# facebookresearch/theseus

Measured on NVIDIA H100. Metric: LM iterations/sec on batched SE3 pose-graph (2500 poses, global batch 2048 over N GPUs, LM + block-sparse Cholesky, fp64), higher is better.
Workload: dtype f64

## Files before the change

### include/thb200.h

```cpp
#ifndef THB200_H_
#define THB200_H_

#include <stdint.h>

#ifdef __cplusplus
extern "C" {
#endif

typedef struct CUstream_st* thb_stream_t;

#define THB_OK 0
#define THB_ERR_BAD_ARG (-1)
#define THB_ERR_UNSUPPORTED (-2)
#define THB_ERR_ALLOC (-3)

int thb_version(void);
int thb_compiled_arch(void);
int64_t thb_launch_count(void);

enum thb_cost_kind {
  THB_COST_BETWEEN_SE3 = 0,
  THB_COST_LOCAL_SE3 = 1,
  THB_COST_BETWEEN_SO3 = 2,
  THB_COST_LOCAL_SO3 = 3,
// ... 260 lines not shown
                       const float* err_prev, const float* err_new, float* lam, int32_t ellipsoidal, float damping_accept,
                       float down_ratio, float up_ratio, uint8_t* reject, float* err_out, int32_t* stats, thb_stream_t stream);

int thb_gram_dense_f64(const double* A, double* AtA, int64_t B, int64_t m, int64_t n, thb_stream_t stream);

typedef struct thb_front_plan {
  int64_t S;
  int64_t n;
  int64_t data_size;
  int64_t arena_size;
  int64_t varena_size;
  const int32_t* f_w; const int32_t* f_b; const int32_t* f_first; const int32_t* f_class;
  const int32_t* f_wpad; const int32_t* f_np; const int32_t* f_cb_ld; const int32_t* f_depth;
  const int64_t* f_panel_off; const int64_t* f_cb_off; const int64_t* f_fr_off; const int64_t* f_u_off;
  const int32_t* child_ptr; const int32_t* child_list;
  const int64_t* rel_ptr; const int32_t* f_rel;
  const int64_t* rows_ptr; const int32_t* f_rows;
  const int32_t* sched;
  const int32_t* perm;
  const int32_t* c_jw; const int64_t* c_sp_ptr; const int32_t* c_sp;
  const int64_t* c_inv_ptr; const int32_t* c_inv;
  const int64_t* fd; const int64_t* pc;
  const int32_t* pmap;
} thb_front_plan;

#define THB_FRONT_LAUNCH_COLS 12
int64_t thb_front_small_smem_bytes(int32_t w, int32_t b, int32_t nchildren);
int thb_front_factor_f64(const thb_front_plan* p, const int64_t* launches, int64_t num_launches, double* factor, const double* ata,
                         int64_t ata_stride, const double* alpha, const double* beta, double* arena, void* dense_ws, int64_t dense_ws_bytes,
                         int32_t* info, int64_t B, thb_stream_t stream);
int thb_front_solve_f64(const thb_front_plan* p, const int64_t* launches, int64_t num_launches, const double* factor, const double* rhs,
                        double* x, double* work, double* varena, int64_t B, thb_stream_t stream);
int thb_front_factor_forward_f64(const thb_front_plan* p, const int64_t* launches, int64_t num_launches, double* factor, const double* ata,
                                 int64_t ata_stride, const double* alpha, const double* beta, double* arena, void* dense_ws,
                                 int64_t dense_ws_bytes, int32_t* info, const double* rhs, double* work, double* varena, int64_t B,
                                 thb_stream_t stream);
int thb_front_forward_f64(const thb_front_plan* p, const int64_t* launches, int64_t num_launches, const double* factor, const double* rhs,
                          double* work, double* varena, int64_t B, thb_stream_t stream);
int thb_front_backward_f64(const thb_front_plan* p, const int64_t* launches, int64_t num_launches, const double* factor, double* x,
                           double* work, int64_t B, thb_stream_t stream);
int64_t thb_potrf_partial_workspace_bytes(int64_t B, int64_t np);
int thb_potrf_partial_inplace_f64(double* F, int64_t bstride, int64_t np, int32_t nb_piv, int32_t w_real, int32_t n_real, int32_t info_base,
                                  int32_t* info, int64_t B, void* workspace, int64_t workspace_bytes, thb_stream_t stream);

int thb_mat_vec_f64(int64_t B, int64_t num_rows, int64_t num_cols, const int64_t* row_ptr, const int64_t* col_ind,
                    const double* A_val, const double* v, double* y, thb_stream_t stream);
// ... 49 lines not shown
```

### theseus_b200/_lib.py

```python
import ctypes as C
import os

_HERE = os.path.dirname(os.path.abspath(__file__))
_LIB_PATH = os.environ.get("THB200_LIB") or os.path.join(_HERE, "lib", "libthb200.so")
_lib = None

c_i32, c_i64, c_f64, c_f32, c_vp = C.c_int32, C.c_int64, C.c_double, C.c_float, C.c_void_p


class CostGroup(C.Structure):
    _fields_ = [("kind", c_i32), ("weight_kind", c_i32), ("K", c_i32), ("dim", c_i32),
                ("x0", c_vp), ("x1", c_vp), ("aux", c_vp), ("w", c_vp), ("bstride", c_vp),
                ("a_off", c_vp), ("a_stride", c_vp), ("bp", c_vp), ("row0", c_vp),
                ("aux2", c_vp), ("aux3", c_vp), ("aux4", c_vp), ("bstride2", c_vp),
                ("robust_kind", c_i32), ("reserved0", c_i32), ("log_radius", c_vp), ("bstride_lr", c_vp),
                ("x2", c_vp), ("x3", c_vp), ("bstride3", c_vp), ("grid_rows", c_i32), ("grid_cols", c_i32)]


class VarTable(C.Structure):
    _fields_ = [("N", c_i32), ("x", c_vp), ("out", c_vp), ("kind", c_vp), ("col", c_vp), ("dof", c_vp)]


_GRAM_STAGED = ("stage_ptr", "st_off", "st_len", "st_row0", "st_dim", "st_soff", "task_ptr", "task_blk", "task_pq", "grp_col", "c_soff",
                "cc_soff", "cc_sb")
# ... 41 lines not shown

_PG, _PV, _PP = C.POINTER(CostGroup), C.POINTER(VarTable), C.POINTER(GramPlan)
_PS = C.POINTER(SparsePlanStruct)
_PL = C.POINTER(SparseLanePlanStruct)


class SparseLaneRootStruct(C.Structure):
    _fields_ = [("num_blocks", c_i64), ("num_cols", c_i64), ("nt", c_i64), ("root_start", c_i64), ("num_segments", c_i64)] + [(k, c_vp) for k in (
        "segments", "rb_off", "rb_row", "rb_col", "rb_di", "rb_dj", "rf_p0", "rf_p1", "root_cols", "root_dims")]


class SparseLaneTilesStruct(C.Structure):
    _fields_ = [("num_tiles", c_i64), ("num_steps", c_i64), ("tile_tgt", c_vp), ("step_ptr", c_vp), ("step_src", c_vp)]


class SparseLanePiecesStruct(C.Structure):
    _fields_ = [("num_pieces", c_i64), ("num_launches", c_i64)] + [(k, c_vp) for k in (
        "launches", "first", "width", "fr_ext_end", "bc_int_end", "order")]


class FrontPlanStruct(C.Structure):
    _fields_ = [("S", c_i64), ("n", c_i64), ("data_size", c_i64), ("arena_size", c_i64), ("varena_size", c_i64)] + [(k, c_vp) for k in (
        "f_w", "f_b", "f_first", "f_class", "f_wpad", "f_np", "f_cb_ld", "f_depth", "f_panel_off", "f_cb_off", "f_fr_off", "f_u_off",
        "child_ptr", "child_list", "rel_ptr", "f_rel", "rows_ptr", "f_rows", "sched", "perm", "c_jw", "c_sp_ptr", "c_sp", "c_inv_ptr", "c_inv", "fd", "pc", "pmap")]


_PF = C.POINTER(FrontPlanStruct)
_PR = C.POINTER(SparseLaneRootStruct)
_PPIECES = C.POINTER(SparseLanePiecesStruct)
_PT = C.POINTER(SparseLaneTilesStruct)
SIGNATURES = {
    "thb_version": (c_i32, []),
    "thb_compiled_arch": (c_i32, []),
    "thb_launch_count": (c_i64, []),
    "thb_linearize_group_f64": (c_i32, [_PG, c_i64, c_vp, c_i64, c_vp, c_i64, c_vp]),
    "thb_linearize_group_f32": (c_i32, [_PG, c_i64, c_vp, c_i64, c_vp, c_i64, c_vp]),
    "thb_error_num_chunks": (c_i32, [c_i32]),
    "thb_error_group_f64": (c_i32, [_PG, c_i64, c_vp, c_vp]),
    "thb_error_group_f32": (c_i32, [_PG, c_i64, c_vp, c_vp]),
    "thb_error_reduce_f64": (c_i32, [c_vp, c_i32, c_i64, c_vp, c_vp]),
    "thb_error_reduce_f32": (c_i32, [c_vp, c_i32, c_i64, c_vp, c_vp]),
    "thb_retract_f64": (c_i32, [_PV, c_i64, c_vp, c_i64, c_f64, c_vp, c_vp]),
    "thb_retract_f32": (c_i32, [_PV, c_i64, c_vp, c_i64, c_f32, c_vp, c_vp]),
    "thb_commit_f64": (c_i32, [_PV, c_i64, c_vp, c_vp]),
    "thb_commit_f32": (c_i32, [_PV, c_i64, c_vp, c_vp]),
    "thb_gram_f64": (c_i32, [_PP, c_i64, c_vp, c_i64, c_vp, c_i64, c_vp, c_i64, c_vp, c_vp, c_vp]),
    "thb_gram_f32": (c_i32, [_PP, c_i64, c_vp, c_i64, c_vp, c_i64, c_vp, c_i64, c_vp, c_vp, c_vp]),
# ... 104 lines not shown
```

### theseus_b200/csrc/thb_front.cu

```cuda
#include <stdlib.h>

#include "thb_common.cuh"

namespace thb {

__device__ __forceinline__ void record_first_failure(int* info, int pos) {
  int old = 0;
  while (true) {
    const int prev = atomicCAS(info, old, pos);
    if (prev == old || (prev != 0 && prev <= pos)) return;
    old = prev;
  }
}

#ifdef THB_SIMT_EMU
#define THB_PDL_TRIGGER() do { } while (0)
#define THB_PDL_WAIT() do { } while (0)
#define FRONT_LAUNCH(K, grid, block, smem, cs, arg) K<<<grid, block, smem, cs>>>(arg)
#else
#define THB_PDL_TRIGGER() asm volatile("griddepcontrol.launch_dependents;" ::: "memory")
#define THB_PDL_WAIT() asm volatile("griddepcontrol.wait;" ::: "memory")
#define FRONT_LAUNCH(K, grid, block, smem, cs, arg) thb::front_launch_pdl(K, grid, block, smem, cs, arg)
static inline bool front_pdl_enabled() {
  static const bool on = [] { const char* e = getenv("THB_FRONT_PDL"); return e != nullptr && e[0] == '1'; }();
// ... 27 lines not shown
  asm volatile("mma.sync.aligned.m8n8k4.row.col.f64.f64.f64.f64 {%0,%1}, {%2}, {%3}, {%0,%1};\n" : "+d"(c0), "+d"(c1) : "d"(a), "d"(b));
}
#endif

__host__ __device__ __forceinline__ int front_pad_ld(int x) { return ((x + 11) / 16) * 16 + 4; }

struct FrontArgs {
  thb_front_plan p;
  int s0;
  int64_t B;
  double* factor;
  const double* alpha;
  const double* beta;
  double* arena_cur;
  const double* arena_child;
  int32_t* info;
  int prefetch;
  const double* ata;
  int64_t ata_stride;
  const double* rhs;
  double* work;
  double* v_cur;
  const double* v_child;
};

__device__ __forceinline__ double front_panel_in(const FrontArgs& a, const double* Lg, int64_t poff, int64_t item, int64_t e) {
  if (a.ata == nullptr) return Lg[e];
  const int32_t m = a.p.pmap[poff + e];
  return m >= 0 ? a.ata[item * a.ata_stride + m] : 0.0;
}

template <typename T>
__device__ __forceinline__ T front_ldg(const T* p) {
#ifdef THB_SIMT_EMU
  return *p;
#else
  return __ldg(p);
#endif
}


constexpr int FRONT_WD_LD = 20;
#ifndef FRONT_PL
#define FRONT_PL 4
#endif
constexpr int FRONT_MAX_CHILDREN = 8;

// ... 230 lines not shown
    i += di; j += dj;
    if (j >= w) { j -= w; i++; }
  }
}

__device__ __forceinline__ void front_store_forward(const FrontArgs& a, const double* U, int ldp, int64_t item, int t, int f_first, int w, int b,
                                                    int tid, int nthreads) {
  for (int i = tid; i < w; i += nthreads) a.work[item * a.p.n + f_first + i] = U[i * ldp];
  double* ub = a.v_cur + item * a.p.varena_size + a.p.f_u_off[t];
  for (int i = tid; i < b; i += nthreads) ub[i] = U[(w + i) * ldp];
}

__host__ __device__ constexpr int front_elim_warps(int threads) { return threads >= 256 ? 4 : threads / 64; }

template <int THREADS>
__global__ void __launch_bounds__(THREADS, 1024 / THREADS) front_small_kernel(FrontArgs a) {
  extern __shared__ double sm[];
  const thb_front_plan& p = a.p;
  const int tid = threadIdx.x, lane = tid & 31, warp = tid >> 5;
  constexpr int NW = THREADS / 32;
  const int lr = lane >> 2, lc = lane & 3;
  const int64_t item = blockIdx.x;
  THB_PDL_TRIGGER();
  const int64_t* FD = p.fd + (int64_t)(a.s0 + blockIdx.y) * 8;
  const int t = (int)FD[0];
  const int w = (int)FD[1], b = (int)FD[2], r = w + b;
  const int f_first = (int)FD[3];
  const int64_t f_panel_off = FD[4];
  const int c_begin = (int)(FD[7] & 0xffffffffLL);
  const int nch = min((int)(FD[7] >> 32), FRONT_MAX_CHILDREN);
  const int b16 = (b + 15) & ~15, w8 = (w + 7) & ~7;
  const int ldp = front_pad_ld(w8);
  const int prow = w8 + b16 + 8;
  double* PN = sm;
  double* Wd = PN + prow * ldp;
  FrontChild* ch = reinterpret_cast<FrontChild*>(Wd + 8 * FRONT_WD_LD);
  int32_t* INV = reinterpret_cast<int32_t*>(Wd + 8 * FRONT_WD_LD + 3 * FRONT_MAX_CHILDREN);
  if (tid < nch) {
    const int64_t* PC = p.pc + (int64_t)(c_begin + tid) * 6;
    ch[tid].src = a.arena_child + item * p.arena_size + PC[0];
    ch[tid].ldg = (int)(PC[1] & 0xffffffffLL);
    ch[tid].lo = (int)PC[2];
    ch[tid].hi = (int)PC[3];
    ch[tid].uoff = (int)PC[5];
  }
  {
// ... 13 lines not shown
  int* next_tile = reinterpret_cast<int*>(Wd + 8);
  if (tid == 0) *next_tile = 0;
  THB_PDL_WAIT();
#ifndef THB_SIMT_EMU
  if (a.rhs != nullptr) {
    for (int i = tid; i < w; i += THREADS) asm volatile("prefetch.global.L2 [%0];\n" ::"l"(a.rhs + item * p.n + p.perm[f_first + i]));
    for (int q = 0; q < nch; q++) {
      const int64_t* PC = p.pc + (int64_t)(c_begin + q) * 6;
      const double* cu = a.v_child + item * p.varena_size + PC[5];
      for (int off = tid * 16; off < (int)(PC[1] >> 32); off += THREADS * 16) asm volatile("prefetch.global.L2 [%0];\n" ::"l"(cu + off));
    }
  }
  for (int q = 0; a.prefetch != 0 && q < nch; q++) {
    const int64_t* PC = p.pc + (int64_t)(c_begin + q) * 6;
    const double* csrc = a.arena_child + item * p.arena_size + PC[0];
    const int cld = (int)(PC[1] & 0xffffffffLL), cbc = (int)(PC[1] >> 32);
    for (int off = tid * 16; off < cbc * cld; off += THREADS * 16) {
      const int i = off / cld, j = off - i * cld;
      if (j <= i) asm volatile("prefetch.global.L2 [%0];\n" ::"l"(csrc + off));
    }
  }
#endif
  __syncthreads();
  if (tid < w8 - w) PN[(w + tid) * ldp + w + tid] = 1.0;
  double* Lg = a.factor + item * p.data_size + f_panel_off;
  {
    const double al = a.alpha != nullptr ? a.alpha[item] : 0.0;
    const double be = a.beta != nullptr ? a.beta[item] : 0.0;
    const int total = r * w;
    for (int e0 = tid; e0 < total; e0 += FRONT_PL * THREADS) {
      int ii[FRONT_PL], jj[FRONT_PL];
      double v[FRONT_PL];
#pragma unroll
      for (int u = 0; u < FRONT_PL; u++) {
        const int e = e0 + u * THREADS;
        ii[u] = e / w;
        jj[u] = e - ii[u] * w;
        if (e >= total || jj[u] > ii[u]) ii[u] = -1;
      }
      int32_t m[FRONT_PL];
#pragma unroll
      for (int u = 0; u < FRONT_PL; u++) m[u] = (a.ata != nullptr && ii[u] >= 0) ? front_ldg(p.pmap + f_panel_off + e0 + u * THREADS) : -1;
      double x[2][FRONT_PL];
      front_panel_gather2(ch, INV, r, nch, 0, ii, jj, x);
#pragma unroll
      for (int u = 0; u < FRONT_PL; u++) {
        if (a.ata != nullptr) v[u] = m[u] >= 0 ? front_ldg(a.ata + item * a.ata_stride + m[u]) : 0.0;
        else v[u] = ii[u] >= 0 ? Lg[e0 + u * THREADS] : 0.0;
      }
#pragma unroll
      for (int u = 0; u < FRONT_PL; u++)
        if (ii[u] >= 0 && ii[u] == jj[u]) v[u] = v[u] + (al * v[u] + be);
      for (int q = 0;;) {
#pragma unroll
        for (int u = 0; u < FRONT_PL; u++) v[u] = (v[u] + x[0][u]) + x[1][u];
        q += 2;
        if (q >= nch) break;
        front_panel_gather2(ch, INV, r, nch, q, ii, jj, x);
      }
#pragma unroll
      for (int u = 0; u < FRONT_PL; u++)
        if (ii[u] >= 0) PN[(ii[u] < w ? ii[u] : ii[u] + (w8 - w)) * ldp + jj[u]] = v[u];
    }
  }
  double* U = PN + w8;
  if (a.rhs != nullptr) {
    for (int i = tid; i < r; i += THREADS) {
      double v = i < w ? a.rhs[item * p.n + p.perm[f_first + i]] : 0.0;
      for (int q = 0; q < nch; q++) {
        if (i >= ch[q].lo && i <= ch[q].hi) {
          const int k = INV[q * r + i];
          if (k >= 0) v += a.v_child[item * p.varena_size + ch[q].uoff + k];
        }
      }
      U[i * ldp] = v;
    }
  }
  __syncthreads();
  const int nbk = w8 / 8, nrt = (w8 + b16) / 8;
  for (int jb = 0; jb < nbk; jb++) {
    if (warp == 0) front_diag_block(PN, ldp, jb, Wd, lane, w, f_first, a.info + item);
    __syncthreads();
    const int npair = (nrt - jb) / 2;
    for (int q = warp; q < npair; q += NW) front_tile_column<true>(PN, ldp, jb, jb + 1 + 2 * q, Wd, lane);
    __syncthreads();
  }
#ifdef THB_SIMT_EMU
  front_store_panel(Lg, PN, ldp, w, w8, r, tid, THREADS);
  if (a.rhs != nullptr) {
    front_forward_elim<THREADS, true>(FrontRowsPanel{PN, ldp, w, w8 - w}, U, ldp, w, r, tid, lane);
    front_store_forward(a, U, ldp, item, t, f_first, w, b, tid, THREADS);
  }
#else
  constexpr int NE = front_elim_warps(THREADS);
  if (a.rhs != nullptr && warp < NE) {
    front_forward_elim<32 * NE, false>(FrontRowsPanel{PN, ldp, w, w8 - w}, U, ldp, w, r, tid, lane);
    front_store_forward(a, U, ldp, item, t, f_first, w, b, tid, 32 * NE);
  } else {
    const int t0 = a.rhs != nullptr ? 32 * NE : 0;
    front_store_panel(Lg, PN, ldp, w, w8, r, tid - t0, THREADS - t0);
  }
#endif
  if (b == 0) return;
  double* dst = a.arena_cur + item * p.arena_size + FD[5];
  const int ldg_out = (int)FD[6];
  const double* P = PN + w8 * ldp;
  const int nmt = b16 / 16;
  for (;;) {
    int q = 0;
    if (lane == 0) q = atomicAdd(next_tile, 1);
    q = __shfl_sync(0xffffffffu, q, 0);
    int R = (int)((sqrtf(8.0f * (float)q + 1.0f) - 1.0f) * 0.5f);
    while ((R + 1) * (R + 2) / 2 <= q) R++;
    while (R * (R + 1) / 2 > q) R--;
    if (R >= nmt) break;
    const int ct = q - R * (R + 1) / 2;
    unsigned reach = 0;
    for (int qc = 0; qc < nch; qc++)
      if (w + 16 * R + 15 >= ch[qc].lo && w + 16 * ct <= ch[qc].hi) reach |= 1u << qc;
    double gch[2][2][2] = {{{-0.0, -0.0}, {-0.0, -0.0}}, {{-0.0, -0.0}, {-0.0, -0.0}}};
    const int li0 = w + 16 * R + lr, lj0 = w + 16 * ct + 2 * lc;
    if (reach != 0) {
      const int qc = front_next_child(reach);
      front_tile_gather(ch[qc], INV + qc * r, r, li0, lj0, gch);
    }
    const bool summed = reach != 0;
// ... 32 lines not shown
          for (int u = 0; u < 2; u++) gch[mi][ni][u] = 0.0 + gch[mi][ni][u];
    }
#pragma unroll
    for (int mi = 0; mi < 2; mi++)
#pragma unroll
      for (int ni = 0; ni < 2; ni++)
#pragma unroll
        for (int u = 0; u < 2; u++) acc[mi][ni][u] = gch[mi][ni][u] - acc[mi][ni][u];
#pragma unroll
    for (int mi = 0; mi < 2; mi++) {
      const int i = 16 * R + 8 * mi + lr;
      if (i < b) {
        double* drow = dst + (int64_t)i * ldg_out;
#pragma unroll
        for (int ni = 0; ni < 2; ni++)
#pragma unroll
          for (int u = 0; u < 2; u++) {
            const int jj = 16 * ct + 8 * ni + 2 * lc + u;
            if (jj <= i) drow[jj] = acc[mi][ni][u];
          }
      }
    }
  }
}

constexpr int ASM_ROWS = 16, ASM_THREADS = 256;

__device__ __forceinline__ int front_map_big(int l, int w, int wpad) { return l < w ? l : wpad + (l - w); }

__global__ void __launch_bounds__(ASM_THREADS, 4) front_assemble_kernel(FrontArgs a, int t) {
  extern __shared__ double sm[];
  const thb_front_plan& p = a.p;
  const int tid = threadIdx.x;
  const int64_t item = blockIdx.x;
  const int w = p.f_w[t], b = p.f_b[t], r = w + b, wpad = p.f_wpad[t], np = p.f_np[t];
  const int R0 = blockIdx.y * ASM_ROWS;
  const int nc = min(np, 128 * (R0 / 128 + 1));
  const int c_first = p.child_ptr[t], n_children = p.child_ptr[t + 1] - c_first;
  if (n_children <= FRONT_MAX_CHILDREN) {
    const double* Lgg = a.factor + item * p.data_size + p.f_panel_off[t];
    const double alg = a.alpha != nullptr ? a.alpha[item] : 0.0;
    const double beg = a.beta != nullptr ? a.beta[item] : 0.0;
    double* Fg = a.arena_cur + item * p.arena_size + p.f_fr_off[t] + (int64_t)R0 * np;
    __shared__ const double* s_src[FRONT_MAX_CHILDREN];
    __shared__ const int32_t* s_inv[FRONT_MAX_CHILDREN];
    __shared__ int s_ld[FRONT_MAX_CHILDREN];
// ... 261 lines not shown
    __syncthreads();
    if (warp == 0) {
      double tk = 0.0;
      if (lane < cw) {
        tk = xf[k0 + lane];
        for (int g = 0; g < RG; g++) tk -= part[g * cw + lane];
      }
      tk = front_warp_trsv_upper(T, tk, cw, lane);
      if (lane < cw) xf[k0 + lane] = tk;
    }
    __syncthreads();
  }
  for (int i = tid; i < w; i += THREADS) {
    const double v = xf[i];
    wk[first + i] = v;
    a.x[item * p.n + p.perm[first + i]] = v;
  }
}

static inline bool front_big_direct() {
  const char* e = getenv("THB_FRONT_BIG_DIRECT");
  return !(e != nullptr && e[0] == '0');
}

static inline int front_threads_of_class(int cls) { return cls == 0 ? 64 : (cls == 1 ? 128 : 256); }

template <typename K>
static inline int front_set_smem(K kernel, size_t bytes, size_t* cache) {
  if (bytes > *cache) {
    cudaError_t e = cudaFuncSetAttribute(kernel, cudaFuncAttributeMaxDynamicSharedMemorySize, (int)bytes);
    if (e != cudaSuccess) return (int)e;
    *cache = bytes;
  }
  return 0;
}

static int front_solve_launch(const thb_front_plan* p, const int64_t* L, int pass, const double* factor, const double* rhs, double* x,
                              double* work, double* varena, int64_t B, cudaStream_t cs) {
  static size_t fw_set[3] = {0, 0, 0}, bw_set[3] = {0, 0, 0};
  static const int64_t stage_cap = [] { const char* e = getenv("THB_SOLVE_STAGE"); return e != nullptr ? (int64_t)atoll(e) : (int64_t)0; }();
  const int depth = (int)L[0], cls = (int)L[1], begin = (int)L[2], count = (int)L[3];
  FrontSolveArgs a;
  a.p = *p; a.s0 = begin; a.B = B; a.factor = factor; a.rhs = rhs; a.x = x; a.work = work;
  a.v_cur = varena != nullptr ? varena + (int64_t)(depth & 1) * B * p->varena_size : nullptr;
  a.v_child = varena != nullptr ? varena + (int64_t)((depth + 1) & 1) * B * p->varena_size : nullptr;
  const int kc = cls > 2 ? 2 : cls;
// ... 19 lines not shown
           FRONT_LAUNCH(front_backward_kernel<256>, grid, 256, smem, cs, a); }
  }
  THB_CHECK_LAUNCH();
  return THB_OK;
}

static int front_factor(const thb_front_plan* p, const int64_t* launches, int64_t num_launches, double* factor, const double* ata,
                        int64_t ata_stride, const double* alpha, const double* beta, double* arena, void* dense_ws, int64_t dense_ws_bytes,
                        int32_t* info, const double* rhs, double* work, double* varena, int64_t B, thb_stream_t stream) {
  if (p == nullptr || launches == nullptr || factor == nullptr || arena == nullptr || info == nullptr || B < 0) return THB_ERR_BAD_ARG;
  if (B == 0 || p->S == 0) return THB_OK;
  if (B > 65535LL * 32768LL) return THB_ERR_UNSUPPORTED;
  cudaStream_t cs = thb_cs(stream);
  THB_CUDA(cudaMemsetAsync(info, 0, (size_t)B * 4, cs));
  static size_t smem_set[5] = {0, 0, 0, 0, 0}, asm_set = 0;
  static const int thr_cls[2] = {[] { const char* e = getenv("THB_FRONT_T0"); const int v = e ? atoi(e) : 64; return (v == 128 || v == 256) ? v : 64; }(),
                                 [] { const char* e = getenv("THB_FRONT_T1"); const int v = e ? atoi(e) : 128; return v == 256 ? 256 : 128; }()};
  static int front_prefetch_flag = -1;
  if (front_prefetch_flag < 0) {
    const char* e = getenv("THB_FRONT_PREFETCH");
    front_prefetch_flag = (e != nullptr && e[0] == '1') ? 1 : 0;
  }
  static const int fuse_max = [] { const char* e = getenv("THB_FRONT_FUSE_MAX"); return e != nullptr ? atoi(e) : 1024; }();
  for (int64_t l = 0; l < num_launches; l++) {
    const int64_t* L = launches + l * THB_FRONT_LAUNCH_COLS;
    const int depth = (int)L[0], cls = (int)L[1], begin = (int)L[2], count = (int)L[3];
    FrontArgs a;
    a.p = *p; a.s0 = begin; a.B = B; a.factor = factor; a.alpha = alpha; a.beta = beta; a.info = info;
    a.ata = (ata != nullptr && p->pmap != nullptr) ? ata : nullptr; a.ata_stride = ata_stride;
    a.prefetch = front_prefetch_flag;
    a.arena_cur = arena + (int64_t)(depth & 1) * B * p->arena_size;
    a.arena_child = arena + (int64_t)((depth + 1) & 1) * B * p->arena_size;
    a.rhs = rhs; a.work = work;
    a.v_cur = rhs != nullptr ? varena + (int64_t)(depth & 1) * B * p->varena_size : nullptr;
    a.v_child = rhs != nullptr ? varena + (int64_t)((depth + 1) & 1) * B * p->varena_size : nullptr;
    if (cls < 3) {
      const size_t smem = (size_t)L[4];
#ifndef THB_SIMT_EMU
      if (smem > 227 * 1024) return THB_ERR_UNSUPPORTED;
#endif
      const dim3 grid((unsigned)B, (unsigned)count);
      if (count > 65535) return THB_ERR_UNSUPPORTED;
      const int threads = (cls == 0 && thr_cls[0] == 64) ? 64
                          : ((cls == 0 && thr_cls[0] == 128) || (cls == 1 && thr_cls[1] == 128)) ? 128
                          : (cls <= 1 || smem <= 56 * 1024) ? 256 : (smem <= 113 * 1024 ? 512 : 1024);
      const bool fused = rhs != nullptr && threads <= fuse_max;
      if (!fused) a.rhs = nullptr;
      if (threads == 64) {
        int rc = front_set_smem(front_small_kernel<64>, smem, &smem_set[0]); if (rc) return rc;
        FRONT_LAUNCH(front_small_kernel<64>, grid, 64, smem, cs, a);
      } else if (threads == 128) {
        int rc = front_set_smem(front_small_kernel<128>, smem, &smem_set[1]); if (rc) return rc;
        FRONT_LAUNCH(front_small_kernel<128>, grid, 128, smem, cs, a);
// ... 42 lines not shown
      front_assemble_kernel<<<dim3((unsigned)B, (unsigned)(np / ASM_ROWS)), ASM_THREADS, smem, cs>>>(a, t);
      THB_CHECK_LAUNCH();
      rc = thb_potrf_partial_inplace_f64(a.arena_cur + fr_off, p->arena_size, np, (int32_t)nb_piv, (int32_t)L[10], n_real,
                                         (int32_t)first, info, B, dense_ws, dense_ws_bytes, stream);
      if (rc != THB_OK) return rc;
      front_extract_kernel<<<dim3((unsigned)B, 8), 256, 0, cs>>>(a, t);
      THB_CHECK_LAUNCH();
      if (rhs != nullptr) {
        rc = front_solve_launch(p, L, 0, factor, rhs, nullptr, work, varena, B, cs);
        if (rc != THB_OK) return rc;
      }
#endif
    }
  }
  return THB_OK;
}

}

extern "C" {

int64_t thb_front_small_smem_bytes(int32_t w, int32_t b, int32_t nchildren) { return thb::front_smem_doubles(w, b, nchildren) * 8; }

int thb_front_factor_f64(const thb_front_plan* p, const int64_t* launches, int64_t num_launches, double* factor, const double* ata,
                         int64_t ata_stride, const double* alpha, const double* beta, double* arena, void* dense_ws, int64_t dense_ws_bytes,
                         int32_t* info, int64_t B, thb_stream_t stream) {
  return thb::front_factor(p, launches, num_launches, factor, ata, ata_stride, alpha, beta, arena, dense_ws, dense_ws_bytes, info, nullptr,
                           nullptr, nullptr, B, stream);
}

int thb_front_factor_forward_f64(const thb_front_plan* p, const int64_t* launches, int64_t num_launches, double* factor, const double* ata,
                                 int64_t ata_stride, const double* alpha, const double* beta, double* arena, void* dense_ws,
                                 int64_t dense_ws_bytes, int32_t* info, const double* rhs, double* work, double* varena, int64_t B,
                                 thb_stream_t stream) {
  if (rhs == nullptr || work == nullptr || varena == nullptr) return THB_ERR_BAD_ARG;
  return thb::front_factor(p, launches, num_launches, factor, ata, ata_stride, alpha, beta, arena, dense_ws, dense_ws_bytes, info, rhs, work,
                           varena, B, stream);
}

int thb_front_solve_f64(const thb_front_plan* p, const int64_t* launches, int64_t num_launches, const double* factor, const double* rhs,
                        double* x, double* work, double* varena, int64_t B, thb_stream_t stream) {
  if (p == nullptr || launches == nullptr || factor == nullptr || rhs == nullptr || x == nullptr || work == nullptr || varena == nullptr ||
      B < 0)
    return THB_ERR_BAD_ARG;
  if (B == 0 || p->S == 0) return THB_OK;
  const int rc = thb_front_forward_f64(p, launches, num_launches, factor, rhs, work, varena, B, stream);
// ... 31 lines not shown
```

### theseus_b200/frontal.py

```python
from dataclasses import dataclass, field
from typing import Dict, List, Optional

import numpy as np

SMALL_CLASSES = (48, 96, 1 << 30)
BIG_TW, BIG_TM = 64, 128


def _bfs_levels(adj, start, mask, stamp, mark):
    mark[start] = True
    levels, seen = [[start]], [start]
    while True:
        nxt = []
        for u in levels[-1]:
            for v in adj[u]:
                if mask[v] == stamp and not mark[v]:
                    mark[v] = True
                    nxt.append(v)
                    seen.append(v)
        if not nxt:
            break
        levels.append(nxt)
    for v in seen:
        mark[v] = False
# ... 143 lines not shown
    col_start: np.ndarray
    perm: np.ndarray
    S: int
    arrays: Dict[str, np.ndarray]
    launches: np.ndarray
    data_size: int
    arena_size: int
    varena_size: int
    stats: Dict[str, float] = field(default_factory=dict)
    front_of_pos: np.ndarray = None
    border_rows: List[np.ndarray] = None

    def gram_compact_offsets(self, blocks_dims):
        f = self.gram_out_offsets()
        pmap = self.arrays["pmap"]
        pmap[:] = -1
        table, off = {}, 0
        for (a, b, di, dj) in blocks_dims:
            po, ld, _ = f(a, b)
            idx = po + np.arange(di)[:, None] * ld + np.arange(dj)[None, :]
            pmap[idx] = off + np.arange(di)[:, None] * dj + np.arange(dj)[None, :]
            table[(a, b)] = (off, dj, -1)
            off += di * dj
        return (lambda a, b: table[(int(a), int(b))]), off

    def gram_out_offsets(self):
        A = self.arrays
        first, w, poff = A["f_first"], A["f_w"], A["f_panel_off"]

        def f(a: int, b: int):
            pa, pb = int(self.pos[a]), int(self.pos[b])
            s = int(self.front_of_pos[pb])
            lcol = int(self.pstart[pb] - first[s])
            ga = int(self.pstart[pa])
            if ga < first[s] + w[s]:
                lrow = ga - int(first[s])
            else:
                k = int(np.searchsorted(self.border_rows[s], ga))
                assert self.border_rows[s][k] == ga
                lrow = int(w[s]) + k
            return int(poff[s]) + lrow * int(w[s]) + lcol, int(w[s]), -1
        return f


def build_front_plan(param_size, ptrs, inds, ordering: str = "auto", tau: float = 0.12, merge_flops: float = 4e4,
                     merge_max_r: int = SMALL_CLASSES[1], small_limit: Optional[int] = None, split_wide: bool = True) -> FrontPlan:
    param_size = np.asarray(param_size, dtype=np.int64)
# ... 263 lines not shown
        i = j
    launches = np.array(launches, dtype=np.int64).reshape(-1, 12)
    fd = np.zeros((max(S, 1), 8), dtype=np.int64)
    pc = np.zeros((max(int(child_ptr[S]), 1), 6), dtype=np.int64)
    for q in range(S):
        t = int(sched[q])
        cb, ce = int(child_ptr[t]), int(child_ptr[t + 1])
        fd[q] = (t, int(f_w[t]), int(f_b[t]), int(f_first[t]), int(f_panel_off[t]), int(f_cb_off[t]), int(f_cb_ld[t]), cb | ((ce - cb) << 32))
    for t in range(S):
        for k, c in enumerate(children[t]):
            rel = f_rel[rel_ptr[c]:rel_ptr[c + 1]]
            pc[int(child_ptr[t]) + k] = (int(f_cb_off[c]), int(f_cb_ld[c]) | (int(f_b[c]) << 32), int(rel[0]), int(rel[-1]), int(c_inv_ptr[c]),
                                         int(f_u_off[c]))
    flops = float(sum(_front_cost(float(f_w[t]), float(f_b[t])) for t in range(S)))
    stats = dict(ordering=oname, column_flops=col_flops, flops=flops, nnz_L=float(sum(int(f_r[t]) * int(f_w[t]) for t in range(S))),
                 fronts=float(S), max_front=float(f_r.max()) if S else 0.0, depth=float(max_depth + 1), big_fronts=float((f_class == 3).sum()),
                 launches=float(len(launches)), cb_doubles=float(sum(int(b) * int(b) for b in f_b)), levels=float(max_depth + 1),
                 num_updates=0.0, num_chains=float(S), chain_levels=float(max_depth + 1))
    arrays = dict(f_w=f_w, f_b=f_b, f_first=f_first, f_parent=f_parent, f_depth=f_depth, f_class=f_class, f_panel_off=f_panel_off,
                  f_wpad=f_wpad, f_np=f_np, f_cb_off=f_cb_off, f_cb_ld=f_cb_ld, f_fr_off=f_fr_off, f_u_off=f_u_off,
                  child_ptr=child_ptr, child_list=np.array(child_list, dtype=np.int32), rel_ptr=rel_ptr, f_rel=f_rel,
                  rows_ptr=rows_ptr, f_rows=f_rows, sched=sched, perm=perm.astype(np.int32), c_jw=c_jw, c_sp_ptr=c_sp_ptr, c_sp=c_sp,
                  c_inv_ptr=c_inv_ptr, c_inv=c_inv, fd=fd.reshape(-1), pc=pc.reshape(-1),
                  pmap=-np.ones(max(int(data_size), 1), dtype=np.int32))
    return FrontPlan(N=N, n=n, param_size=param_size, order=order, pos=pos, dims=dims, pstart=pstart, col_start=col_start, perm=perm, S=S,
                     arrays=arrays, launches=launches, data_size=int(data_size), arena_size=int(arena_size), varena_size=int(varena_size),
                     stats=stats, front_of_pos=front_of_pos, border_rows=border_rows)


def execute_numpy(plan: FrontPlan, panels: np.ndarray, rhs: np.ndarray):
    A = plan.arrays
    P = panels.astype(np.float64).copy()
    S = plan.S
    cb: Dict[int, np.ndarray] = {}
    w, b, first, poff = A["f_w"], A["f_b"], A["f_first"], A["f_panel_off"]

    def rel_of(c):
        return A["f_rel"][A["rel_ptr"][c]:A["rel_ptr"][c + 1]]

    def kids(t):
        return A["child_list"][A["child_ptr"][t]:A["child_ptr"][t + 1]]
    for (d, cls, s0, cnt) in plan.launches[:, :4]:
        for t in A["sched"][s0:s0 + cnt]:
            wt, bt = int(w[t]), int(b[t])
            r = wt + bt
            F = np.zeros((r, r))
            F[:, :wt] = P[poff[t]:poff[t] + r * wt].reshape(r, wt)
# ... 40 lines not shown
```

### theseus_b200/sparse_solver.py

```python
import ctypes as C
import os
from typing import Any, Dict, Optional, Type, Union

import numpy as np
import torch

from . import _lib
from .autograd import LinearSolveFunction, wants_grad
from .core import Objective
from .optimizer import (Linearization, LinearSolver, SparseLinearization, convert_to_alpha_beta_damping_tensors)
from .frontal import build_front_plan
from .sparse import ITEM_MAX_DIM, LANE_DIMS, analyze, gram_out_offsets, piece_solve_lists, root_lane_lists, root_split, tile_lane_lists
from .structure import ata_block_structure, build_gram_plan


_ROOT_LAYOUTS = ("lane_root", "lane_tiled_root")
_TILED_LAYOUTS = ("lane_tiled", "lane_tiled_root")


class BaspachoSparseSolver(LinearSolver):
    def __init__(self, objective: Objective, linearization_cls: Optional[Type[Linearization]] = None,
                 linearization_kwargs: Optional[Dict[str, Any]] = None, num_solver_contexts=1, batch_size: Optional[int] = None,
                 auto_reset: bool = True, dev: Optional[str] = None, ordering: str = "mindeg", layout: Optional[str] = None,
                 supernodal_solve: bool = False, front_options: Optional[Dict[str, Any]] = None, **kwargs):
# ... 129 lines not shown
            tl, tt = self._tile_lists()
            tst, tdev, tlaunch = self._lane_struct(tl, dev, device)
            ttdev = {k: torch.from_numpy(np.ascontiguousarray(v)).to(device) for k, v in tt.items()}
            tiles = _lib.SparseLaneTilesStruct(num_tiles=int(tt["tile_tgt"].shape[0]), num_steps=int(tt["step_src"].shape[0]),
                                               tile_tgt=ttdev["tile_tgt"].data_ptr(), step_ptr=ttdev["step_ptr"].data_ptr(),
                                               step_src=ttdev["step_src"].data_ptr())
            self._dev.update({self._layout: tst}, tiles=tiles, tkeep=(tdev, tlaunch, ttdev))
        if getattr(self, "_supernodal_solve", False) and all(int(d) in LANE_DIMS for d in P.dims):
            ps = piece_solve_lists(P, cut=self._root_split()[0]["cut"] if self._layout in _ROOT_LAYOUTS else None)
            pdev = {k: torch.from_numpy(np.ascontiguousarray(ps[k] if k != "width" else ps[k].astype(np.int32))).to(device)
                    for k in ("first", "width", "fr_ext_end", "bc_int_end", "order")}
            plaunch = np.ascontiguousarray(ps["launches"][:, 1:], dtype=np.int32)
            pst = _lib.SparseLanePiecesStruct(num_pieces=int(ps["first"].shape[0]), num_launches=int(plaunch.shape[0]), launches=plaunch.ctypes.data,
                                              **{k: pdev[k].data_ptr() for k in pdev})
            self._dev.update(pieces=pst, pkeep=(pdev, plaunch, ps))
        return self._dev

    def _device_plan_front(self, device):
        P = self._plan
        dev = {k: torch.from_numpy(np.ascontiguousarray(v)).to(device) for k, v in P.arrays.items()}
        st = _lib.FrontPlanStruct(S=P.S, n=P.n, data_size=P.data_size, arena_size=P.arena_size, varena_size=P.varena_size,
                                  **{k: dev[k].data_ptr() for k in ("f_w", "f_b", "f_first", "f_class", "f_wpad", "f_np", "f_cb_ld", "f_depth",
                                                                    "f_panel_off", "f_cb_off", "f_fr_off", "f_u_off", "child_ptr", "child_list",
                                                                    "rel_ptr", "f_rel", "rows_ptr", "f_rows", "sched", "perm", "c_jw", "c_sp_ptr", "c_sp", "c_inv_ptr", "c_inv", "fd", "pc", "pmap")})
        g = self._gram_arrays
        gdev = {k: torch.from_numpy(np.ascontiguousarray(v)).to(device) for k, v in g.items() if isinstance(v, np.ndarray)}
        launches = np.ascontiguousarray(P.launches, dtype=np.int64)
        big = launches[launches[:, 1] == 3]
        self._dev = dict(device=device, front=st, keep=dev, gram=_lib.make_gram_plan(g, gdev), gkeep=gdev, bufs={}, launches=launches,
                         max_np=int(big[:, 5].max()) if len(big) else 0)
        return self._dev

    def _numeric_front(self, A_val, b, alpha, beta, forward=False):
        B, device = A_val.shape[0], A_val.device
        d = self._device_plan(device)
        P = self._plan
        lib = _lib.load()
        s = _lib.stream_ptr()
        chunk = int(min(B, self._front_options.get("chunk", int(os.environ.get("THB_FRONT_CHUNK", "1024")))))
        if d["bufs"].get("key") != (B, "front"):
            ws_bytes = int(lib.thb_potrf_partial_workspace_bytes(chunk, d["max_np"])) if d["max_np"] else 0
            d["bufs"] = dict(key=(B, "front"), chunk=chunk, factor=torch.empty(B, P.data_size, dtype=torch.float64, device=device),
                             ata=torch.empty(B, self._ata_size, dtype=torch.float64, device=device),
                             arena=torch.empty(2, chunk, P.arena_size, dtype=torch.float64, device=device),
                             varena=torch.empty(2, chunk, P.varena_size, dtype=torch.float64, device=device),
                             work=torch.empty(B, P.n, dtype=torch.float64, device=device),
                             ws=torch.empty(max(ws_bytes, 8), dtype=torch.uint8, device=device),
# ... 223 lines not shown
```

Before: 5.790.

## Stage AtA panel entries into shared memory with precomputed cp.async copy runs

Adds a host-built list of copy runs that maps gram (AtA) entries straight to front-panel shared-memory positions, pairing adjacent aligned entries into 16-byte copies. The small-front kernel fills the panel with cp.async instead of a per-element pmap indirection. Leaf fronts with no children skip the general gather loop and only apply the LM damping to the diagonal. It also adds optional compile-time phase timers. The cost is extra plan arrays, an env toggle (on by default), and a full wait on the async copies before the panel is used.

```diff
diff --git a/include/thb200.h b/include/thb200.h
--- a/include/thb200.h
+++ b/include/thb200.h
@@ -306,6 +306,8 @@
   const int64_t* c_inv_ptr; const int32_t* c_inv;
   const int64_t* fd; const int64_t* pc;
   const int32_t* pmap;
+  const int64_t* arun_ptr;
+  const int32_t* arun;
 } thb_front_plan;
 
 #define THB_FRONT_LAUNCH_COLS 12
diff --git a/theseus_b200/_lib.py b/theseus_b200/_lib.py
--- a/theseus_b200/_lib.py
+++ b/theseus_b200/_lib.py
@@ -87,7 +87,7 @@
 class FrontPlanStruct(C.Structure):
     _fields_ = [("S", c_i64), ("n", c_i64), ("data_size", c_i64), ("arena_size", c_i64), ("varena_size", c_i64)] + [(k, c_vp) for k in (
         "f_w", "f_b", "f_first", "f_class", "f_wpad", "f_np", "f_cb_ld", "f_depth", "f_panel_off", "f_cb_off", "f_fr_off", "f_u_off",
-        "child_ptr", "child_list", "rel_ptr", "f_rel", "rows_ptr", "f_rows", "sched", "perm", "c_jw", "c_sp_ptr", "c_sp", "c_inv_ptr", "c_inv", "fd", "pc", "pmap")]
+        "child_ptr", "child_list", "rel_ptr", "f_rel", "rows_ptr", "f_rows", "sched", "perm", "c_jw", "c_sp_ptr", "c_sp", "c_inv_ptr", "c_inv", "fd", "pc", "pmap", "arun_ptr", "arun")]
 
 
 _PF = C.POINTER(FrontPlanStruct)
diff --git a/theseus_b200/csrc/thb_front.cu b/theseus_b200/csrc/thb_front.cu
--- a/theseus_b200/csrc/thb_front.cu
+++ b/theseus_b200/csrc/thb_front.cu
@@ -73,7 +73,45 @@
   double* work;
   double* v_cur;
   const double* v_child;
+  int stage_ata;
+#ifdef THB_FRONT_PHASE_CLOCKS
+  unsigned long long* clocks;
+  int clock_every;
+  int clock_items;
+#endif
 };
+
+#ifndef THB_SIMT_EMU
+__device__ __forceinline__ void front_cp_async_8(double* smem_dst, const double* gmem_src) {
+  asm volatile("cp.async.ca.shared.global [%0], [%1], 8;" ::"r"((unsigned)__cvta_generic_to_shared(smem_dst)), "l"(gmem_src) : "memory");
+}
+__device__ __forceinline__ void front_cp_async_16(double* smem_dst, const double* gmem_src) {
+  asm volatile("cp.async.cg.shared.global [%0], [%1], 16;" ::"r"((unsigned)__cvta_generic_to_shared(smem_dst)), "l"(gmem_src) : "memory");
+}
+__device__ __forceinline__ void front_cp_async_wait_all() { asm volatile("cp.async.commit_group;\ncp.async.wait_all;" ::: "memory"); }
+#else
+inline void front_cp_async_8(double* smem_dst, const double* gmem_src) { *smem_dst = *gmem_src; }
+inline void front_cp_async_16(double* smem_dst, const double* gmem_src) { smem_dst[0] = gmem_src[0]; smem_dst[1] = gmem_src[1]; }
+inline void front_cp_async_wait_all() {}
+#endif
+
+#ifdef THB_FRONT_PHASE_CLOCKS
+__device__ __forceinline__ unsigned long long front_globaltimer() {
+  unsigned long long t;
+  asm volatile("mov.u64 %0, %globaltimer;" : "=l"(t));
+  return t;
+}
+#define FRONT_CLOCK(k)                                                                                                             \
+  do {                                                                                                                             \
+    if (a.clocks != nullptr && item % a.clock_every == 0 && item / a.clock_every < a.clock_items) {                                \
+      unsigned long long* ck = a.clocks + ((int64_t)(a.s0 + blockIdx.y) * a.clock_items + item / a.clock_every) * 6;                \
+      if ((k) < 4 && tid == 0) ck[k] = front_globaltimer();                                                                        \
+      if ((k) >= 4 && lane == 0) atomicMax(ck + (k), front_globaltimer());                                                         \
+    }                                                                                                                              \
+  } while (0)
+#else
+#define FRONT_CLOCK(k) do { } while (0)
+#endif
 
 __device__ __forceinline__ double front_panel_in(const FrontArgs& a, const double* Lg, int64_t poff, int64_t item, int64_t e) {
   if (a.ata == nullptr) return Lg[e];
@@ -350,6 +388,7 @@
   const int lr = lane >> 2, lc = lane & 3;
   const int64_t item = blockIdx.x;
   THB_PDL_TRIGGER();
+  FRONT_CLOCK(0);
   const int64_t* FD = p.fd + (int64_t)(a.s0 + blockIdx.y) * 8;
   const int t = (int)FD[0];
   const int w = (int)FD[1], b = (int)FD[2], r = w + b;
@@ -409,13 +448,43 @@
   }
 #endif
   __syncthreads();
+  FRONT_CLOCK(1);
+  const bool staged = a.stage_ata != 0;
+  if (staged) {
+    const double* src = a.ata + item * a.ata_stride;
+    const bool src16 = (reinterpret_cast<uintptr_t>(src) & 15) == 0;
+    const int64_t* runs = reinterpret_cast<const int64_t*>(p.arun);
+    const int run0 = (int)p.arun_ptr[a.s0 + blockIdx.y], run1 = (int)p.arun_ptr[a.s0 + blockIdx.y + 1];
+    for (int k0 = run0 + tid; k0 < run1; k0 += FRONT_PL * THREADS) {
+      int64_t pc[FRONT_PL];
+#pragma unroll
+      for (int u = 0; u < FRONT_PL; u++) pc[u] = k0 + u * THREADS < run1 ? front_ldg(runs + k0 + u * THREADS) : (int64_t)-1;
+#pragma unroll
+      for (int u = 0; u < FRONT_PL; u++) {
+        const int so = (int)(pc[u] & 0xffffffffLL), dc = (int)(pc[u] >> 32);
+        if (dc < 0) continue;
+        double* d = PN + (dc >> 1);
+        if (!(dc & 1)) front_cp_async_8(d, src + so);
+        else if (src16) front_cp_async_16(d, src + so);
+        else { front_cp_async_8(d, src + so); front_cp_async_8(d + 1, src + so + 1); }
+      }
+    }
+    front_cp_async_wait_all();
+    __syncthreads();
+  }
   if (tid < w8 - w) PN[(w + tid) * ldp + w + tid] = 1.0;
   double* Lg = a.factor + item * p.data_size + f_panel_off;
   {
     const double al = a.alpha != nullptr ? a.alpha[item] : 0.0;
     const double be = a.beta != nullptr ? a.beta[item] : 0.0;
     const int total = r * w;
-    for (int e0 = tid; e0 < total; e0 += FRONT_PL * THREADS) {
+    if (staged && nch == 0) {
+      for (int i = tid; i < w; i += THREADS) {
+        const double v = PN[i * ldp + i];
+        PN[i * ldp + i] = v + (al * v + be);
+      }
+    }
+    for (int e0 = tid; e0 < ((staged && nch == 0) ? 0 : total); e0 += FRONT_PL * THREADS) {
       int ii[FRONT_PL], jj[FRONT_PL];
       double v[FRONT_PL];
 #pragma unroll
@@ -427,12 +496,13 @@
       }
       int32_t m[FRONT_PL];
 #pragma unroll
-      for (int u = 0; u < FRONT_PL; u++) m[u] = (a.ata != nullptr && ii[u] >= 0) ? front_ldg(p.pmap + f_panel_off + e0 + u * THREADS) : -1;
+      for (int u = 0; u < FRONT_PL; u++) m[u] = (!staged && a.ata != nullptr && ii[u] >= 0) ? front_ldg(p.pmap + f_panel_off + e0 + u * THREADS) : -1;
       double x[2][FRONT_PL];
       front_panel_gather2(ch, INV, r, nch, 0, ii, jj, x);
 #pragma unroll
       for (int u = 0; u < FRONT_PL; u++) {
-        if (a.ata != nullptr) v[u] = m[u] >= 0 ? front_ldg(a.ata + item * a.ata_stride + m[u]) : 0.0;
+        if (staged) v[u] = ii[u] >= 0 ? PN[(ii[u] < w ? ii[u] : ii[u] + (w8 - w)) * ldp + jj[u]] : 0.0;
+        else if (a.ata != nullptr) v[u] = m[u] >= 0 ? front_ldg(a.ata + item * a.ata_stride + m[u]) : 0.0;
         else v[u] = ii[u] >= 0 ? Lg[e0 + u * THREADS] : 0.0;
       }
 #pragma unroll
@@ -464,6 +534,7 @@
     }
   }
   __syncthreads();
+  FRONT_CLOCK(2);
   const int nbk = w8 / 8, nrt = (w8 + b16) / 8;
   for (int jb = 0; jb < nbk; jb++) {
     if (warp == 0) front_diag_block(PN, ldp, jb, Wd, lane, w, f_first, a.info + item);
@@ -472,6 +543,7 @@
     for (int q = warp; q < npair; q += NW) front_tile_column<true>(PN, ldp, jb, jb + 1 + 2 * q, Wd, lane);
     __syncthreads();
   }
+  FRONT_CLOCK(3);
 #ifdef THB_SIMT_EMU
   front_store_panel(Lg, PN, ldp, w, w8, r, tid, THREADS);
   if (a.rhs != nullptr) {
@@ -488,7 +560,8 @@
     front_store_panel(Lg, PN, ldp, w, w8, r, tid - t0, THREADS - t0);
   }
 #endif
-  if (b == 0) return;
+  FRONT_CLOCK(4);
+  if (b == 0) { FRONT_CLOCK(5); return; }
   double* dst = a.arena_cur + item * p.arena_size + FD[5];
   const int ldg_out = (int)FD[6];
   const double* P = PN + w8 * ldp;
@@ -567,6 +640,7 @@
       }
     }
   }
+  FRONT_CLOCK(5);
 }
 
 constexpr int ASM_ROWS = 16, ASM_THREADS = 256;
@@ -874,6 +948,16 @@
   const char* e = getenv("THB_FRONT_BIG_DIRECT");
   return !(e != nullptr && e[0] == '0');
 }
+
+static inline bool front_stage_ata() {
+  const char* e = getenv("THB_FRONT_STAGE_ATA");
+  return !(e != nullptr && e[0] == '0');
+}
+
+#ifdef THB_FRONT_PHASE_CLOCKS
+static unsigned long long* front_clock_buf = nullptr;
+static int front_clock_every = 1, front_clock_items = 0;
+#endif
 
 static inline int front_threads_of_class(int cls) { return cls == 0 ? 64 : (cls == 1 ? 128 : 256); }
 
@@ -939,6 +1023,7 @@
     front_prefetch_flag = (e != nullptr && e[0] == '1') ? 1 : 0;
   }
   static const int fuse_max = [] { const char* e = getenv("THB_FRONT_FUSE_MAX"); return e != nullptr ? atoi(e) : 1024; }();
+  const int stage_ata = (ata != nullptr && p->pmap != nullptr && p->arun_ptr != nullptr && p->arun != nullptr && front_stage_ata()) ? 1 : 0;
   for (int64_t l = 0; l < num_launches; l++) {
     const int64_t* L = launches + l * THB_FRONT_LAUNCH_COLS;
     const int depth = (int)L[0], cls = (int)L[1], begin = (int)L[2], count = (int)L[3];
@@ -946,6 +1031,10 @@
     a.p = *p; a.s0 = begin; a.B = B; a.factor = factor; a.alpha = alpha; a.beta = beta; a.info = info;
     a.ata = (ata != nullptr && p->pmap != nullptr) ? ata : nullptr; a.ata_stride = ata_stride;
     a.prefetch = front_prefetch_flag;
+    a.stage_ata = stage_ata;
+#ifdef THB_FRONT_PHASE_CLOCKS
+    a.clocks = front_clock_buf; a.clock_every = front_clock_every; a.clock_items = front_clock_items;
+#endif
     a.arena_cur = arena + (int64_t)(depth & 1) * B * p->arena_size;
     a.arena_child = arena + (int64_t)((depth + 1) & 1) * B * p->arena_size;
     a.rhs = rhs; a.work = work;
@@ -1034,6 +1123,12 @@
 
 int64_t thb_front_small_smem_bytes(int32_t w, int32_t b, int32_t nchildren) { return thb::front_smem_doubles(w, b, nchildren) * 8; }
 
+#ifdef THB_FRONT_PHASE_CLOCKS
+void thb_front_phase_clocks(unsigned long long* buf, int32_t every, int32_t items) {
+  thb::front_clock_buf = buf; thb::front_clock_every = every > 0 ? every : 1; thb::front_clock_items = items;
+}
+#endif
+
 int thb_front_factor_f64(const thb_front_plan* p, const int64_t* launches, int64_t num_launches, double* factor, const double* ata,
                          int64_t ata_stride, const double* alpha, const double* beta, double* arena, void* dense_ws, int64_t dense_ws_bytes,
                          int32_t* info, int64_t B, thb_stream_t stream) {
diff --git a/theseus_b200/frontal.py b/theseus_b200/frontal.py
--- a/theseus_b200/frontal.py
+++ b/theseus_b200/frontal.py
@@ -189,7 +189,41 @@
             pmap[idx] = off + np.arange(di)[:, None] * dj + np.arange(dj)[None, :]
             table[(a, b)] = (off, dj, -1)
             off += di * dj
+        self.ata_copy_pieces()
         return (lambda a, b: table[(int(a), int(b))]), off
+
+    def ata_copy_pieces(self):
+        A = self.arrays
+        pmap, sched = A["pmap"], A["sched"]
+        f_w, f_b, f_panel_off = A["f_w"], A["f_b"], A["f_panel_off"]
+        ptr = np.zeros(self.S + 1, dtype=np.int64)
+        runs = []
+        for q in range(self.S):
+            t = int(sched[q])
+            if A["f_class"][t] == 3:
+                ptr[q + 1] = ptr[q]
+                continue
+            w, r = int(f_w[t]), int(f_w[t]) + int(f_b[t])
+            w8 = (w + 7) & ~7
+            ldp = ((w8 + 11) // 16) * 16 + 4
+            e = np.arange(r * w, dtype=np.int64)
+            i, j = e // w, e % w
+            m = pmap[int(f_panel_off[t]) + e].astype(np.int64)
+            keep = (m >= 0) & ((i >= w) | (j <= i))
+            i, j, m = i[keep], j[keep], m[keep]
+            dst = np.where(i < w, i, i + (w8 - w)) * ldp + j
+            nxt = np.zeros(len(dst), dtype=bool)
+            nxt[:-1] = (dst[1:] == dst[:-1] + 1) & (m[1:] == m[:-1] + 1)
+            wide = nxt & (dst % 2 == 0) & (m % 2 == 0)
+            second = np.zeros(len(dst), dtype=bool)
+            second[1:] = wide[:-1]
+            sel = ~second
+            runs.append(np.stack([m[sel], (dst[sel] << 1) | wide[sel]], axis=1))
+            ptr[q + 1] = ptr[q] + int(sel.sum())
+        arun = np.concatenate(runs) if runs else np.zeros((0, 2), dtype=np.int64)
+        assert arun.size == 0 or (arun.max() < 2 ** 31 and arun.min() >= 0)
+        A["arun_ptr"] = ptr
+        A["arun"] = np.ascontiguousarray(arun if len(arun) else np.zeros((1, 2), dtype=np.int64), dtype=np.int32).reshape(-1)
 
     def gram_out_offsets(self):
         A = self.arrays
@@ -499,7 +533,8 @@
                   child_ptr=child_ptr, child_list=np.array(child_list, dtype=np.int32), rel_ptr=rel_ptr, f_rel=f_rel,
                   rows_ptr=rows_ptr, f_rows=f_rows, sched=sched, perm=perm.astype(np.int32), c_jw=c_jw, c_sp_ptr=c_sp_ptr, c_sp=c_sp,
                   c_inv_ptr=c_inv_ptr, c_inv=c_inv, fd=fd.reshape(-1), pc=pc.reshape(-1),
-                  pmap=-np.ones(max(int(data_size), 1), dtype=np.int32))
+                  pmap=-np.ones(max(int(data_size), 1), dtype=np.int32),
+                  arun_ptr=np.zeros(S + 1, dtype=np.int64), arun=np.zeros(2, dtype=np.int32))
     return FrontPlan(N=N, n=n, param_size=param_size, order=order, pos=pos, dims=dims, pstart=pstart, col_start=col_start, perm=perm, S=S,
                      arrays=arrays, launches=launches, data_size=int(data_size), arena_size=int(arena_size), varena_size=int(varena_size),
                      stats=stats, front_of_pos=front_of_pos, border_rows=border_rows)
diff --git a/theseus_b200/sparse_solver.py b/theseus_b200/sparse_solver.py
--- a/theseus_b200/sparse_solver.py
+++ b/theseus_b200/sparse_solver.py
@@ -175,7 +175,8 @@
         st = _lib.FrontPlanStruct(S=P.S, n=P.n, data_size=P.data_size, arena_size=P.arena_size, varena_size=P.varena_size,
                                   **{k: dev[k].data_ptr() for k in ("f_w", "f_b", "f_first", "f_class", "f_wpad", "f_np", "f_cb_ld", "f_depth",
                                                                     "f_panel_off", "f_cb_off", "f_fr_off", "f_u_off", "child_ptr", "child_list",
-                                                                    "rel_ptr", "f_rel", "rows_ptr", "f_rows", "sched", "perm", "c_jw", "c_sp_ptr", "c_sp", "c_inv_ptr", "c_inv", "fd", "pc", "pmap")})
+                                                                    "rel_ptr", "f_rel", "rows_ptr", "f_rows", "sched", "perm", "c_jw", "c_sp_ptr", "c_sp", "c_inv_ptr", "c_inv", "fd", "pc", "pmap", "arun_ptr",
+                                                                    "arun")})
         g = self._gram_arrays
         gdev = {k: torch.from_numpy(np.ascontiguousarray(v)).to(device) for k, v in g.items() if isinstance(v, np.ndarray)}
         launches = np.ascontiguousarray(P.launches, dtype=np.int64)
```

After: 5.872, median of 6. 1.4% higher.
